# TaKeTube/TaKe

Measured on AMD Instinct MI355X. Metric: Msamples/s (camera paths/s: rays traced x spp / s), 1M-tri soup; weak scaling: 256 spp per GPU, higher is better.
Workload: dtype f64+f32; 1 GPU; procedural 1000000-triangle soup (diffuse materials) in 5-wall box + 1 quad area light, 1920x1080, 256 spp per GPU (256 total), max_depth 50, no Russian roulette, procedural sky env-map 2048x1024, importance-sampled (extension); parallelism=tile-row strips over 1 GPU(s), scene replicated, one gather

## Files before the change

### take_amd/csrc/tk_adaptive.h

```cpp
#pragma once
#include <cstdint>

#include "tk_integrate.h"

namespace tk {
namespace ad {

struct Rule {
    int32_t spp, min_spp, step_spp;
    double threshold, floor;
};

TK_HD double sample_value(double r, double g, double b) { return (r + g) + b; }
TK_HD void add_moments(double L, double &m1, double &m2) {
    m1 = m1 + L;
    m2 = m2 + L * L;
}

TK_HD double rel_error(int32_t n, double m1, double m2, double floor) {
    const double dn = (double)n;
    const double mean = m1 / dn;
    double v = m2 / dn - mean * mean;
    v = v > 0.0 ? v : 0.0;
    return tk_sqrt(v / (dn - 1.0)) / (tk_fabs(mean) + floor);
// ... 27 lines not shown
        base[g] = prefix;
        prefix += bits_of(mask[g]);
    }
    return prefix;
}
TK_HD int32_t compact_dest(const uint64_t *mask, const int32_t *base, int64_t j) {
    return base[j / GROUP] + rank_below(mask[j / GROUP], (int)(j % GROUP));
}

inline int32_t compact_serial(const uint8_t *keep, const int32_t *list, int64_t n, int threads, uint64_t *mask, int32_t *base, int32_t *out) {
    const int64_t n_groups = groups_of(n);
    for (int64_t g = 0; g < n_groups; g++) {
        uint64_t m = 0;
        for (int l = 0; l < GROUP; l++)
            if (g * GROUP + l < n && keep[g * GROUP + l]) m |= 1ull << l;
        mask[g] = m;
    }
    int32_t prefix = 0;
    for (int t = 0; t < threads; t++) {
        int64_t lo, hi;
        scan_run(n_groups, threads, t, lo, hi);
        prefix = run_number(mask, lo, hi, prefix, base);
    }
    for (int64_t j = 0; j < n; j++)
        if (kept(mask[j / GROUP], (int)(j % GROUP))) out[compact_dest(mask, base, j)] = listed(list, j);
    return prefix;
}

#if defined(__HIPCC__)

template <class R>
__global__ void __launch_bounds__(BLOCK)
k_generate_list(DeviceScene<R> sc, RenderParams<R> rp, PathState<R> st, const int32_t *__restrict__ list, int32_t n_active, double inv_n_active,
                int32_t *queue, int64_t n) {
    for (int64_t j = (int64_t)blockIdx.x * BLOCK + threadIdx.x; j < n; j += (int64_t)gridDim.x * BLOCK) {
        uint32_t sample, idx;
        list_entry((uint32_t)j, (uint32_t)n_active, inv_n_active, sample, idx);
        const int64_t slot = slot_of(sample, list[idx], rp.npix);
        generate_path(sc, rp, st, slot);
        queue[j] = (int32_t)slot;
    }
}

template <class R>
__global__ void __launch_bounds__(BLOCK)
k_accumulate_stats(PathState<R> st, R *accum, int32_t *count, double *m1, double *m2, const int32_t *__restrict__ list, int32_t n_active,
                   int32_t npix, int32_t nb) {
    for (int32_t j = blockIdx.x * BLOCK + threadIdx.x; j < n_active; j += gridDim.x * BLOCK) {
        const int32_t p = listed(list, j);
        R r = accum[3 * (int64_t)p], g = accum[3 * (int64_t)p + 1], b = accum[3 * (int64_t)p + 2];
        double s1 = m1[p], s2 = m2[p];
        for (int s = 0; s < nb; s++) {
            const int64_t slot = slot_of((uint32_t)s, p, npix);
            const R lr = st.R_(S_LX, slot), lg = st.R_(S_LY, slot), lb = st.R_(S_LZ, slot);
            r = r + lr;
            g = g + lg;
            b = b + lb;
            add_moments(sample_value((double)lr, (double)lg, (double)lb), s1, s2);
        }
        accum[3 * (int64_t)p] = r;
        accum[3 * (int64_t)p + 1] = g;
        accum[3 * (int64_t)p + 2] = b;
        m1[p] = s1, m2[p] = s2;
        count[p] += nb;
    }
}
__global__ void __launch_bounds__(BLOCK)
k_accumulate_stats_mixed(PathState<double> a, PathState<float> b, double *accum, int32_t *count, double *m1, double *m2,
                         const int32_t *__restrict__ list, int32_t n_active, int32_t npix, int32_t nb) {
    for (int32_t j = blockIdx.x * BLOCK + threadIdx.x; j < n_active; j += gridDim.x * BLOCK) {
        const int32_t p = listed(list, j);
        double r = accum[3 * (int64_t)p], g = accum[3 * (int64_t)p + 1], bl = accum[3 * (int64_t)p + 2];
        double s1 = m1[p], s2 = m2[p];
        for (int s = 0; s < nb; s++) {
            const int64_t slot = slot_of((uint32_t)s, p, npix);
            const bool conv = a.I_(S_CONV, slot) != 0;
            const float bx = b.R_(S_LX, slot), by = b.R_(S_LY, slot), bz = b.R_(S_LZ, slot);
            const double lr = a.R_(S_LX, slot) + (conv ? (double)bx : 0.0);
            const double lg = a.R_(S_LY, slot) + (conv ? (double)by : 0.0);
            const double lb = a.R_(S_LZ, slot) + (conv ? (double)bz : 0.0);
            r = r + lr;
            g = g + lg;
            bl = bl + lb;
            add_moments(sample_value(lr, lg, lb), s1, s2);
        }
        accum[3 * (int64_t)p] = r;
        accum[3 * (int64_t)p + 1] = g;
        accum[3 * (int64_t)p + 2] = bl;
        m1[p] = s1, m2[p] = s2;
        count[p] += nb;
    }
}

__global__ void __launch_bounds__(BLOCK)
k_adaptive_select(Rule rule, const int32_t *__restrict__ count, const double *__restrict__ m1, const double *__restrict__ m2,
                  const int32_t *__restrict__ list, int32_t n_active, uint64_t *mask) {
    const int64_t j = (int64_t)blockIdx.x * BLOCK + threadIdx.x;
    bool keep = false;
    if (j < n_active) {
        const int32_t p = listed(list, j);
        const int32_t n = count[p];
        keep = !stops(rule, n, rel_error(n, m1[p], m2[p], rule.floor));
    }
    const uint64_t m = __ballot(keep);
    if (lane_id() == 0 && j < n_active) mask[j / GROUP] = m;
}
__global__ void __launch_bounds__(SCAN_THREADS) k_compact_scan(const uint64_t *__restrict__ mask, int64_t n_groups, int32_t *base, int32_t *n_next) {
    __shared__ int32_t s_sum[SCAN_THREADS];
    int64_t lo, hi;
    scan_run(n_groups, SCAN_THREADS, (int)threadIdx.x, lo, hi);
    const int32_t sum = run_sum(mask, lo, hi);
    s_sum[threadIdx.x] = sum;
    __syncthreads();
    for (int off = 1; off < SCAN_THREADS; off <<= 1) {
        const int32_t v = (int)threadIdx.x >= off ? s_sum[threadIdx.x - off] : 0;
        __syncthreads();
        s_sum[threadIdx.x] += v;
        __syncthreads();
    }
    (void)run_number(mask, lo, hi, s_sum[threadIdx.x] - sum, base);
    if (threadIdx.x == SCAN_THREADS - 1) *n_next = s_sum[SCAN_THREADS - 1];
}
__global__ void __launch_bounds__(BLOCK)
k_compact_scatter(const int32_t *__restrict__ list, const uint64_t *__restrict__ mask, const int32_t *__restrict__ base, int32_t n_active,
                  int32_t *next) {
    for (int64_t j = (int64_t)blockIdx.x * BLOCK + threadIdx.x; j < n_active; j += (int64_t)gridDim.x * BLOCK)
        if (kept(mask[j / GROUP], (int)(j % GROUP))) next[compact_dest(mask, base, j)] = listed(list, j);
}

template <class R>
__global__ void __launch_bounds__(BLOCK)
k_resolve_adaptive(const R *__restrict__ accum, const int32_t *__restrict__ count, const double *__restrict__ m1, const double *__restrict__ m2, R *out,
                   int32_t *count_out, double *m1_out, double *m2_out, int32_t width, int32_t n_local_rows) {
// ... 19 lines not shown
```

### take_amd/csrc/tk_integrate.h

```cpp
#pragma once

#include "tk_shade.h"

namespace tk {

template <class R> struct RenderParams {
    int32_t width, height;
    int32_t n_local_rows;
    int32_t npix;
    int32_t strip_first, strip_stride;
    int32_t spp;
    int32_t s0;
    int32_t spb;
    int32_t max_depth;
    int32_t integrator;
    uint64_t seed;
    R ray_eps;
    double inv_npix, inv_width;
};

TK_HD void divmod_u31(uint32_t n, uint32_t d, double inv_d, uint32_t &q, uint32_t &r) {
    if (inv_d == 0.0) {
        q = n / d, r = n % d;
        return;
// ... 5 lines not shown
}
template <class R> TK_HD void slot_pixel(const RenderParams<R> &rp, int64_t slot, int &sl, int &lr, int &x) {
    uint32_t q, p, row, col;
    divmod_u31((uint32_t)slot, (uint32_t)rp.npix, rp.inv_npix, q, p);
    divmod_u31(p, (uint32_t)rp.width, rp.inv_width, row, col);
    sl = (int)q, lr = (int)row, x = (int)col;
}

constexpr int TILE_ROWS = 4;

template <class R> TK_HD int local_row_to_y(const RenderParams<R> &rp, int lr) {
    return (rp.strip_first + (lr / TILE_ROWS) * rp.strip_stride) * TILE_ROWS + (lr % TILE_ROWS);
}

template <class R> TK_HD Rng path_rng(const RenderParams<R> &rp, int64_t slot, uint32_t ctr) {
    int sl, lr, x;
    slot_pixel(rp, slot, sl, lr, x);
    const int y = local_row_to_y(rp, lr);
    Rng r;
    r.key = rng_key(rp.seed, (uint64_t)y * (uint64_t)rp.width + (uint64_t)x, (uint64_t)(rp.s0 + sl));
    r.ctr = ctr;
    return r;
}

constexpr uint32_t CAMERA_DRAWS = 2;
template <class R> TK_HD Vec3<R> camera_dir(const CameraRec<R> &c, const RenderParams<R> &rp, int64_t slot) {
    int sl, lr, x;
    slot_pixel(rp, slot, sl, lr, x);
    const int y = local_row_to_y(rp, lr);
    Rng rng = path_rng(rp, slot, 0);
    const R ry = random_real<R>(rng);
    const R rx = random_real<R>(rng);
    return normalize(ld3(c.u) * ((R(x) + rx) / R(c.width) - R(0.5)) * c.viewport_width +
                     ld3(c.v) * ((R(y) + ry) / R(c.height) - R(0.5)) * c.viewport_height - ld3(c.w));
}
template <class R>
TK_HD void generate_path(const DeviceScene<R> &sc, const RenderParams<R> &rp, const PathState<R> &st, int64_t slot) {
    const CameraRec<R> &c = sc.cam;
    const Vec3<R> d = camera_dir(c, rp, slot);
    Rng rng = path_rng(rp, slot, 0);
    rng.ctr = CAMERA_DRAWS;
    st.R_(S_OX, slot) = c.lookfrom[0];
    st.R_(S_OY, slot) = c.lookfrom[1];
    st.R_(S_OZ, slot) = c.lookfrom[2];
    st.R_(S_DX, slot) = d.x;
    st.R_(S_DY, slot) = d.y;
    st.R_(S_DZ, slot) = d.z;
    st.R_(S_TX, slot) = R(1);
    st.R_(S_TY, slot) = R(1);
    st.R_(S_TZ, slot) = R(1);
    st.R_(S_LX, slot) = R(0);
    st.R_(S_LY, slot) = R(0);
    st.R_(S_LZ, slot) = R(0);
    st.I_(S_CTR, slot) = (int32_t)rng.ctr;
    st.I_(S_FLAGS, slot) = 0;
    st.I_(S_OCC, slot) = -1;
    st.I_(S_CONV, slot) = 0;
}

constexpr uint32_t REQ_EXTEND = 1, REQ_SHADOW = 2;
constexpr int TAG_ANY = -1;
constexpr int TAG_MISS = TAKE_MAT_COUNT;

template <class R, int TAG = TAG_ANY, class ST = PathState<R>>
TK_HD uint32_t shade_path(const DeviceScene<R> &sc, const RenderParams<R> &rp, const ST &st, int64_t slot,
                          int k) {
    const int32_t hit_prim = st.I_(S_HIT, slot);
    const Vec3<R> ro{st.R_(S_OX, slot), st.R_(S_OY, slot), st.R_(S_OZ, slot)};
    const Vec3<R> rd{st.R_(S_DX, slot), st.R_(S_DY, slot), st.R_(S_DZ, slot)};
    Vec3<R> thr{st.R_(S_TX, slot), st.R_(S_TY, slot), st.R_(S_TZ, slot)};
    Vec3<R> rad{st.R_(S_LX, slot), st.R_(S_LY, slot), st.R_(S_LZ, slot)};
    if (k == 0) {
        thr = Vec3<R>{R(1), R(1), R(1)};
        rad = Vec3<R>{R(0), R(0), R(0)};
        if (sizeof(R) == 8) st.I_(S_CONV, slot) = 0;
    }
    const Vec3<R> bg = ld3(sc.background);
    const R nlights = R(sc.n_lights);
    const bool miss = (TAG == TAG_MISS) || hit_prim < 0;
    Isect<R> v{};
    bool alive = !miss;
    if (!miss) make_isect(sc, ro, rd, hit_prim, st.R_(S_HT, slot), st.R_(S_HU, slot), st.R_(S_HV, slot), v,
                            sc.inst_shade ? st.I_(S_INST, slot) : -1);

    if (k == 0) {
        if (miss) {
            rad = bg;
            if (sc.env.light >= 0) {
                R unused;
                rad = env_eval(sc, rd, unused);
            }
        } else if (v.area_light != -1) {
            const LightRec<R> &l = sc.lights[v.area_light];
            if (l.kind == 1) rad = rad + thr * ld3(l.intensity);
        }
    } else {
        const Vec3<R> FG{st.R_(S_FX, slot), st.R_(S_FY, slot), st.R_(S_FZ, slot)};
        const R pdf = st.R_(S_PDF, slot);
        const bool was_specular = (st.I_(S_FLAGS, slot) & FLAG_SPECULAR) != 0;
        if (miss && sc.env.light >= 0) {
            R env_pdf;
            const Vec3<R> L = env_eval(sc, rd, env_pdf);
            const R light_pdf = env_pdf / nlights;
            rad = rad + thr * (FG * L * (was_specular ? (R(1) / pdf) : (pdf / (light_pdf * light_pdf + pdf * pdf))));
            thr = thr * (FG / pdf);
        } else if (miss) {
            thr = thr * (FG / pdf);
            rad = rad + thr * bg;
        } else {
            Vec3<R> C2{R(0), R(0), R(0)};
            if (v.area_light != -1) {
                const LightRec<R> &l = sc.lights[v.area_light];
                const R d = length(v.pos - ro);
                const Vec3<R> light_dir = normalize(v.pos - ro);
                const R light_pdf =
                    light_pdf_area(l, v.pos, ro) * (d * d) / (tk_fmax(dot(-v.gn, light_dir), R(0)) * nlights);
                if (light_pdf <= R(0)) {
                    alive = false;
                } else if (l.kind == 1) {
                    C2 = FG * ld3(l.intensity) *
                         (was_specular ? (R(1) / pdf) : (pdf / (light_pdf * light_pdf + pdf * pdf)));
                }
            }
            if (alive) {
                rad = rad + thr * C2;
                thr = thr * (FG / pdf);
            }
        }
    }
// ... 62 lines not shown
                const Vec3<R> dir_out = normalize(rec.dir_out);
                if (rec.pdf > R(0)) {
                    st.R_(S_DX, slot) = dir_out.x;
                    st.R_(S_DY, slot) = dir_out.y;
                    st.R_(S_DZ, slot) = dir_out.z;
                    st.R_(S_FX, slot) = FG.x;
                    st.R_(S_FY, slot) = FG.y;
                    st.R_(S_FZ, slot) = FG.z;
                    st.R_(S_PDF, slot) = rec.pdf;
                    st.I_(S_FLAGS, slot) = is_specular ? FLAG_SPECULAR : 0;
                    req |= REQ_EXTEND;
                }
            }
        }
        st.R_(S_OX, slot) = v.pos.x;
        st.R_(S_OY, slot) = v.pos.y;
        st.R_(S_OZ, slot) = v.pos.z;
        st.I_(S_CTR, slot) = (int32_t)rng.ctr;
    }
    st.R_(S_TX, slot) = thr.x;
    st.R_(S_TY, slot) = thr.y;
    st.R_(S_TZ, slot) = thr.z;
    st.R_(S_LX, slot) = rad.x;
    st.R_(S_LY, slot) = rad.y;
    st.R_(S_LZ, slot) = rad.z;
    return req;
}

constexpr int32_t FLAG_LIGHT_BRANCH = 2;
constexpr int FLAG_ITER_SHIFT = 8;

template <class R, class G> TK_HD int sample_light_by_power(const DeviceScene<R> &sc, G &rng) {
    const R u = random_real<R>(rng);
    const int size = sc.n_lights;
    int lo = 0, hi = size + 1;
    while (lo < hi) {
        const int mid = (lo + hi) >> 1;
        if (sc.light_cdf[mid] > u) hi = mid;
        else lo = mid + 1;
    }
    const int off = lo - 1;
    return off < 0 ? 0 : (off > size - 1 ? size - 1 : off);
}

template <class R, int TAG = TAG_ANY, class ST = PathState<R>>
TK_HD uint32_t shade_path_alt(const DeviceScene<R> &sc, const RenderParams<R> &rp, const ST &st, int64_t slot,
                              int k) {
    const bool raw = rp.integrator == 1, power = rp.integrator == 3;
    const int32_t hit_prim = st.I_(S_HIT, slot);
    const Vec3<R> ro{st.R_(S_OX, slot), st.R_(S_OY, slot), st.R_(S_OZ, slot)};
    const Vec3<R> rd{st.R_(S_DX, slot), st.R_(S_DY, slot), st.R_(S_DZ, slot)};
    Vec3<R> thr{st.R_(S_TX, slot), st.R_(S_TY, slot), st.R_(S_TZ, slot)};
    Vec3<R> rad{st.R_(S_LX, slot), st.R_(S_LY, slot), st.R_(S_LZ, slot)};
    const Vec3<R> bg = ld3(sc.background);
    const R nlights = R(sc.n_lights);
    const bool miss = (TAG == TAG_MISS) || hit_prim < 0;
    Isect<R> v{};
    if (!miss) make_isect(sc, ro, rd, hit_prim, st.R_(S_HT, slot), st.R_(S_HU, slot), st.R_(S_HV, slot), v,
                            sc.inst_shade ? st.I_(S_INST, slot) : -1);
    const int32_t flags = st.I_(S_FLAGS, slot);
    int iter = flags >> FLAG_ITER_SHIFT;
    bool alive = true;
    if (k == 0) {
        iter = 0;
        if (miss) rad = bg, alive = false;
    } else {
        const Vec3<R> FG{st.R_(S_FX, slot), st.R_(S_FY, slot), st.R_(S_FZ, slot)};
        const R pdf = st.R_(S_PDF, slot);
        if (raw) {
            if (miss) rad = rad + thr * bg, alive = false;
        } else if (flags & FLAG_LIGHT_BRANCH) {
            if (miss) {
                if (power) rad = rad + thr * bg;
                alive = false;
            } else if (power && v.area_light == -1) {
                alive = false;
            } else {
                thr = thr * (FG / pdf);
            }
        } else {
            const bool was_specular = (flags & FLAG_SPECULAR) != 0;
            R p = (sc.n_lights == 0 || was_specular) ? pdf : R(0.5) * pdf;
            if (miss) {
                thr = thr * (FG / p);
                rad = rad + thr * bg;
                alive = false;
            } else {
                if (!was_specular && v.area_light != -1) {
                    const LightRec<R> &l = sc.lights[v.area_light];
                    const R d = length(v.pos - ro);
                    const Vec3<R> light_dir = normalize(v.pos - ro);
                    const R lpd = light_pdf_area(l, v.pos, ro) * (d * d);
                    const R light_pdf = power ? lpd * sc.light_pmf[v.area_light] / tk_fmax(dot(-v.gn, light_dir), R(0))
                                              : lpd / (tk_fmax(dot(-v.gn, light_dir), R(0)) * nlights);
                    if (light_pdf <= R(0)) alive = false;
                    else p = p + R(0.5) * light_pdf;
                }
                if (alive) thr = thr * (FG / p);
            }
        }
        iter++;
    }

    uint32_t req = 0;
    if (TAG != TAG_MISS && alive) {
        Rng rng = path_rng(rp, slot, (uint32_t)st.I_(S_CTR, slot));
// ... 60 lines not shown
```

### take_amd/csrc/tk_kernels.h

```cpp
#pragma once

#include <hip/hip_runtime.h>

#include "tk_integrate.h"
#include "tk_trace_quad.h"

namespace tk {

constexpr int BLOCK = 256;
constexpr int WAVE = 64;

__device__ __forceinline__ int lane_id() { return threadIdx.x & (WAVE - 1); }
__device__ __forceinline__ int mask_rank(uint64_t mask) {
    return __builtin_amdgcn_mbcnt_hi((uint32_t)(mask >> 32), __builtin_amdgcn_mbcnt_lo((uint32_t)mask, 0));
}
__device__ __forceinline__ void wave_append(bool want, int32_t value, int32_t *counter, int32_t *queue) {
    const uint64_t mask = __ballot(want);
    if (mask == 0) return;
    const int leader = __ffsll((unsigned long long)mask) - 1;
    int32_t base = 0;
    if (lane_id() == leader) base = atomicAdd(counter, (int32_t)__popcll(mask));
    base = __shfl(base, leader);
    if (want) queue[base + mask_rank(mask)] = value;
}

template <class R>
__global__ void __launch_bounds__(BLOCK)
k_generate(DeviceScene<R> sc, RenderParams<R> rp, PathState<R> st, int32_t *queue, int64_t n) {
    for (int64_t s = (int64_t)blockIdx.x * BLOCK + threadIdx.x; s < n; s += (int64_t)gridDim.x * BLOCK) {
        generate_path(sc, rp, st, s);
        queue[s] = (int32_t)s;
    }
}

template <class R> struct CameraIo : PathIo<R> {
    CameraRec<R> cam;
    RenderParams<R> rp;
    template <bool SHADOW> __device__ __forceinline__ void load(int32_t i, RayT<R> &ray, int32_t &tag) const {
        const int64_t slot = i;
        tag = i;
        const Vec3<R> d = camera_dir(cam, rp, slot);
        const PathState<R> &st = this->st;
        st.R_(S_OX, slot) = cam.lookfrom[0], st.R_(S_OY, slot) = cam.lookfrom[1], st.R_(S_OZ, slot) = cam.lookfrom[2];
        st.R_(S_DX, slot) = d.x, st.R_(S_DY, slot) = d.y, st.R_(S_DZ, slot) = d.z;
        ray = make_ray(cam.lookfrom[0], cam.lookfrom[1], cam.lookfrom[2], d.x, d.y, d.z, this->eps, Const<R>::inf());
    }
};
__global__ void __launch_bounds__(BLOCK) k_iota(int32_t *queue, int64_t n) {
    for (int64_t s = (int64_t)blockIdx.x * BLOCK + threadIdx.x; s < n; s += (int64_t)gridDim.x * BLOCK) queue[s] = (int32_t)s;
}

#ifndef TK_SHADE_RECORD
#define TK_SHADE_RECORD 1
#endif
template <class R> struct RecordView {
    union {
        mutable uint4 q[PATH_REC * sizeof(R) / 16];
        mutable R w[PATH_REC];
    };
    __device__ __forceinline__ RecordView() {}
    __device__ __forceinline__ R &R_(int c, int64_t) const { return w[c]; }
    __device__ __forceinline__ int32_t &I_(int c, int64_t) const { return *reinterpret_cast<int32_t *>(&w[c]); }
};
#ifndef TK_SHADE_WAVES_F32
#define TK_SHADE_WAVES_F32 5
#endif
#ifndef TK_SHADE_WAVES_F64
#define TK_SHADE_WAVES_F64 0
#endif
template <class R, int TAG, bool ALT> constexpr int shade_waves() {
    const bool lambert = TAG == 0 || TAG == 7 || TAG == 8 || TAG == 10 || TAG == 11;
    const int w = sizeof(R) == 4 ? ((lambert && !ALT) ? TK_SHADE_WAVES_F32 : 0) : TK_SHADE_WAVES_F64;
    return w > 0 ? w : 1;
}
template <class R, int TAG, bool ALT = false>
__global__ void __launch_bounds__(BLOCK, (shade_waves<R, TAG, ALT>()))
k_shade(DeviceScene<R> sc, RenderParams<R> rp, PathState<R> st, const int32_t *__restrict__ queue,
        const int32_t *__restrict__ n_ptr, const int32_t *__restrict__ tag_count, int32_t *next_queue,
        int32_t *n_next, int32_t *shadow_queue, int32_t *n_shadow, int k, unsigned long long *counters, float *to_f32) {
    int32_t begin = 0, n = *n_ptr;
    if (tag_count) {
        for (int t = 0; t < TAG; t++) begin += tag_count[t];
        n = tag_count[TAG];
    }
    if (blockIdx.x == 0 && threadIdx.x == 0) atomicAdd(&counters[C_BOUNCES], (unsigned long long)n);
    const int32_t i = blockIdx.x * BLOCK + threadIdx.x;
    if (blockIdx.x * BLOCK >= n) return;
    uint32_t req = 0;
    int32_t slot = 0;
    if (i < n) {
        slot = queue[begin + i];
#if TK_SHADE_RECORD
        if constexpr (sizeof(R) == 4) {
            RecordView<R> rv;
            const char *rec = (const char *)(st.r + (int64_t)slot * PATH_REC);
            asm volatile(
                "global_load_dwordx4 %0, %8, off\n\t"
                "global_load_dwordx4 %1, %8, off offset:16\n\t"
                "global_load_dwordx4 %2, %8, off offset:32\n\t"
                "global_load_dwordx4 %3, %8, off offset:48\n\t"
                "global_load_dwordx4 %4, %8, off offset:64\n\t"
                "global_load_dwordx4 %5, %8, off offset:80\n\t"
                "global_load_dwordx4 %6, %8, off offset:96\n\t"
                "global_load_dwordx4 %7, %8, off offset:112\n\t"
                "s_waitcnt vmcnt(0)"
                : "=&v"(rv.q[0]), "=&v"(rv.q[1]), "=&v"(rv.q[2]), "=&v"(rv.q[3]), "=&v"(rv.q[4]), "=&v"(rv.q[5]), "=&v"(rv.q[6]),
                  "=&v"(rv.q[7])
                : "v"(rec)
                : "memory");
            req = ALT ? shade_path_alt<R, TAG, RecordView<R>>(sc, rp, rv, (int64_t)slot, k)
                      : shade_path<R, TAG, RecordView<R>>(sc, rp, rv, (int64_t)slot, k);
            uint4 *out = (uint4 *)(st.r + (int64_t)slot * PATH_REC);
#pragma unroll
            for (int c = 0; c < PATH_REC / 4; c++) out[c] = rv.q[c];
        } else
#endif
#if TK_SHADE_RECORD
        if constexpr (sizeof(R) == 8) {
            RecordView<R> rv;
            const char *rec = (const char *)(st.r + (int64_t)slot * PATH_REC);
            asm volatile(
                "global_load_dwordx4 %0, %16, off\n\t"
                "global_load_dwordx4 %1, %16, off offset:16\n\t"
                "global_load_dwordx4 %2, %16, off offset:32\n\t"
                "global_load_dwordx4 %3, %16, off offset:48\n\t"
// ... 114 lines not shown
    for (int32_t i = lo; i < hi; i++) sum += hist[i];
    s_sum[threadIdx.x] = sum;
    __syncthreads();
    for (int off = 1; off < SORT_SCAN_THREADS; off <<= 1) {
        const int32_t v = threadIdx.x >= off ? s_sum[threadIdx.x - off] : 0;
        __syncthreads();
        s_sum[threadIdx.x] += v;
        __syncthreads();
    }
    int32_t run = s_sum[threadIdx.x] - sum;
    for (int32_t i = lo; i < hi; i++) {
        base[i] = run;
        run += hist[i];
    }
    __syncthreads();
    if (threadIdx.x < N_SORT_KEYS) {
        const int32_t first = threadIdx.x * n_waves, next = first + n_waves;
        const int32_t end = next < total ? base[next] : s_sum[SORT_SCAN_THREADS - 1];
        tag_count[threadIdx.x] = end - base[first];
    }
}
__global__ void __launch_bounds__(BLOCK)
k_sort_scatter(const int32_t *__restrict__ queue, const int32_t *__restrict__ n_ptr, const uint8_t *__restrict__ keys,
               const int32_t *__restrict__ base, int32_t *sorted) {
    const int32_t n = *n_ptr, n_waves = gridDim.x * (BLOCK / WAVE);
    const int32_t w = blockIdx.x * (BLOCK / WAVE) + threadIdx.x / WAVE;
    int32_t begin, end;
    sort_range(n, w, n_waves, begin, end);
    if (begin >= end) return;
    int32_t off[N_SORT_KEYS];
#pragma unroll
    for (int t = 0; t < N_SORT_KEYS; t++) off[t] = base[t * n_waves + w];
    for (int32_t i = begin + lane_id(); i < end + lane_id(); i += WAVE) {
        const bool valid = i < end;
        const int key = valid ? (int)keys[i] : -1;
        int32_t pos = 0;
#pragma unroll
        for (int t = 0; t < N_SORT_KEYS; t++) {
            const uint64_t m = __ballot(key == t);
            if (key == t) pos = off[t] + mask_rank(m);
            off[t] += (int32_t)__popcll(m);
        }
        if (valid) sorted[pos] = queue[i];
    }
}

template <class R>
__global__ void __launch_bounds__(BLOCK)
k_accumulate(PathState<R> st, R *accum, int32_t npix, int32_t spb) {
    for (int32_t p = blockIdx.x * BLOCK + threadIdx.x; p < npix; p += gridDim.x * BLOCK) {
        R r = accum[3 * (int64_t)p], g = accum[3 * (int64_t)p + 1], b = accum[3 * (int64_t)p + 2];
        for (int s = 0; s < spb; s++) {
            const int64_t slot = (int64_t)s * npix + p;
            r = r + st.R_(S_LX, slot);
            g = g + st.R_(S_LY, slot);
            b = b + st.R_(S_LZ, slot);
        }
        accum[3 * (int64_t)p] = r;
        accum[3 * (int64_t)p + 1] = g;
        accum[3 * (int64_t)p + 2] = b;
    }
}
__global__ void __launch_bounds__(BLOCK)
k_convert_state(PathState<double> a, PathState<float> b, const int32_t *__restrict__ queue, const int32_t *__restrict__ n_ptr) {
    const int32_t n = *n_ptr;
    for (int32_t i = blockIdx.x * BLOCK + threadIdx.x; i < n; i += gridDim.x * BLOCK) {
        const int64_t s = queue[i];
        constexpr int WORDS[] = {S_OX, S_OY, S_OZ, S_DX, S_DY, S_DZ, S_PDF, S_TX, S_TY, S_TZ, S_LX, S_LY, S_LZ, S_FX, S_FY, S_FZ};
#pragma unroll
        for (int w = 0; w < 16; w++) b.R_(WORDS[w], s) = (float)a.R_(WORDS[w], s);
        b.I_(S_CTR, s) = a.I_(S_CTR, s);
        b.I_(S_FLAGS, s) = a.I_(S_FLAGS, s);
        b.I_(S_OCC, s) = -1;
        a.R_(S_LX, s) = 0.0, a.R_(S_LY, s) = 0.0, a.R_(S_LZ, s) = 0.0;
        a.I_(S_CONV, s) = 1;
    }
}
__global__ void __launch_bounds__(BLOCK)
k_accumulate_mixed(PathState<double> a, PathState<float> b, double *accum, int32_t npix, int32_t spb) {
    for (int32_t p = blockIdx.x * BLOCK + threadIdx.x; p < npix; p += gridDim.x * BLOCK) {
        double r = accum[3 * (int64_t)p], g = accum[3 * (int64_t)p + 1], bl = accum[3 * (int64_t)p + 2];
        for (int s = 0; s < spb; s++) {
            const int64_t slot = (int64_t)s * npix + p;
            const bool conv = a.I_(S_CONV, slot) != 0;
            const float bx = b.R_(S_LX, slot), by = b.R_(S_LY, slot), bz = b.R_(S_LZ, slot);
            r = r + (a.R_(S_LX, slot) + (conv ? (double)bx : 0.0));
            g = g + (a.R_(S_LY, slot) + (conv ? (double)by : 0.0));
            bl = bl + (a.R_(S_LZ, slot) + (conv ? (double)bz : 0.0));
        }
        accum[3 * (int64_t)p] = r;
        accum[3 * (int64_t)p + 1] = g;
        accum[3 * (int64_t)p + 2] = bl;
    }
}
template <class R>
__global__ void __launch_bounds__(BLOCK)
k_resolve(const R *__restrict__ accum, R *out, int32_t width, int32_t n_local_rows, int32_t spp) {
    const int32_t npix = width * n_local_rows;
    const R inv = R(1) / R(spp);
    for (int32_t p = blockIdx.x * BLOCK + threadIdx.x; p < npix; p += gridDim.x * BLOCK) {
        const int lr = p / width, x = p % width;
        const int64_t o = 3 * ((int64_t)(n_local_rows - 1 - lr) * width + x);
        out[o] = accum[3 * (int64_t)p] * inv;
        out[o + 1] = accum[3 * (int64_t)p + 1] * inv;
        out[o + 2] = accum[3 * (int64_t)p + 2] * inv;
    }
}

__device__ __forceinline__ uint16_t exr_half_bits(float f) {
    const uint32_t u = __float_as_uint(f);
    const uint32_t sign = (u >> 16) & 0x8000u;
    const int32_t exp = (int32_t)((u >> 23) & 0xFFu);
    const uint32_t man = u & 0x7FFFFFu;
    const int32_t newexp = exp - 112;
    uint32_t out = 0;
    if (exp == 255) out = 0x7C00u | (man != 0 ? 0x200u : 0u);
    else if (exp != 0 && newexp >= 31) out = 0x7C00u;
    else if (exp != 0 && newexp > 0) out = (((uint32_t)newexp << 10) | (man >> 13)) + ((man >> 12) & 1u);
    else if (exp != 0 && 14 - newexp <= 24) {
        const uint32_t full = man | 0x800000u;
        const int sh = 14 - newexp;
        out = (full >> sh) + ((full >> (sh - 1)) & 1u);
    }
    return (uint16_t)(out | sign);
}
template <class R>
__global__ void __launch_bounds__(BLOCK) k_pack_exr(const R *__restrict__ rgb, int32_t width, int32_t height, uint16_t *out) {
    const int64_t total = (int64_t)width * height * 3;
    for (int64_t i = (int64_t)blockIdx.x * BLOCK + threadIdx.x; i < total; i += (int64_t)gridDim.x * BLOCK) {
        const int x = (int)(i % width);
        const int c = (int)((i / width) % 3);
        const int64_t y = i / ((int64_t)3 * width);
        out[i] = exr_half_bits((float)rgb[(y * width + x) * 3 + (2 - c)]);
    }
}

}

namespace tk {
enum DebugTable { TAB_MATERIAL = 0, TAB_LIGHT = 1, TAB_TEXTURE = 2, TAB_TO_WORLD = 3, TAB_HEMICOS = 4, TAB_BURLEY = 5 };
constexpr int TAB_RND = 8;
// ... 98 lines not shown
```

### take_amd/csrc/tk_scene.h

```cpp
#pragma once

#include "tk_common.h"

namespace tk {

constexpr int32_t CHILD_EMPTY = (int32_t)0x80000000;
constexpr int MAX_LEAF = 4;
constexpr int MAX_STACK_ENTRIES_W8 = 192;
constexpr int MAX_STACK_ENTRIES = 96;

TK_HD int32_t make_leaf(int32_t first, int32_t count) { return -(1 + first * MAX_LEAF + (count - 1)); }
TK_HD int32_t leaf_first(int32_t c) { return (-c - 1) / MAX_LEAF; }
TK_HD int32_t leaf_count(int32_t c) { return ((-c - 1) % MAX_LEAF) + 1; }
constexpr int32_t INSTANCE_WORD_END = -(1 << 30);
TK_HD int32_t make_instance_word(int32_t id) { return (int32_t)(0x80000001u + (uint32_t)id); }
TK_HD bool is_instance_word(int32_t c) { return c < INSTANCE_WORD_END && c != CHILD_EMPTY; }
TK_HD int32_t instance_of_word(int32_t c) { return (int32_t)((uint32_t)c - 0x80000001u); }

template <class R> struct alignas(16) NodeChild {
    R bmin[3];
    R bmax[3];
    int32_t child;
    int32_t pad;
};
// ... 94 lines not shown
};

template <class R> struct alignas(16) InstTrace {
    R inv[12];
    float grid_lo[3], grid_step[3];
    int32_t root_child;
    int32_t pad;
};
template <class R> struct alignas(16) InstShade {
    R fwd[9];
    int32_t material;
    int32_t tag;
    int32_t shape_base;
    int32_t pad;
};

template <class R> struct CameraRec {
    R u[3], v[3], w[3], lookfrom[3];
    R viewport_width, viewport_height;
    int32_t width, height;
};

template <class R> struct DeviceScene {
    const Node4<R> *nodes;
    const QNode4 *qnodes;
    const QNode8 *qnodes8;
    float grid_lo[3], grid_step[3];
    const PrimRec<R> *prims;
    int32_t root_child;
    int32_t n_nodes;
    const ShapeInfo *shapes;
    const MeshInfo *meshes;
    const int32_t *face_idx;
    const R *normals;
    const R *uvs;
    const MaterialRec<R> *materials;
    const ImageInfo *images;
    const R *texels;
    const InstTrace<R> *inst_trace;
    const InstShade<R> *inst_shade;
    int32_t n_instances;
    const LightRec<R> *lights;
    const R *light_pmf;
    const R *light_cdf;
    int32_t n_lights;
    int32_t n_shapes;
    R background[3];
    EnvMap<R> env;
    CameraRec<R> cam;
};

enum StateR {
    S_OX = 0, S_OY, S_OZ,
    S_DX, S_DY, S_DZ,
    S_HT, S_HU, S_HV,
    S_PDF = 12,
    S_TX, S_TY, S_TZ,
    S_LX, S_LY, S_LZ,
    S_ST,
    S_FX, S_FY, S_FZ,
    S_SX, S_SY, S_SZ,
    S_CX, S_CY, S_CZ,
    S_NUM_R = 29
};
enum StateI { S_HIT = 9, S_CTR = 10, S_FLAGS = 11, S_INST = 29, S_OCC = 30, S_CONV = 31, S_NUM_I = 6 };
constexpr int PATH_REC = 32;
constexpr int32_t FLAG_SPECULAR = 1;

template <class R> struct PathState {
    R *r;
    int64_t stride;
    TK_HD R &R_(int c, int64_t s) const { return r[s * PATH_REC + c]; }
    TK_HD int32_t &I_(int c, int64_t s) const { return *reinterpret_cast<int32_t *>(&r[s * PATH_REC + c]); }
};

enum QueueWord {
    Q_N_EXT0, Q_N_EXT1,
    Q_N_SHADOW,
    Q_HEAD_CLOSEST,
    Q_HEAD_SHADOW,
    Q_HEAD_SHADE,
    Q_NUM_WORDS = 16
};

enum CounterWord {
    C_NODE_VISITS, C_PRIM_TESTS, C_RAYS_CLOSEST, C_RAYS_SHADOW, C_BOUNCES, C_LEAF_VISITS, C_WAVE_NODE_STEPS,
    C_WAVE_LEAF_STEPS, C_WAIT_SLOTS, C_IDLE_SLOTS,
    C_RAYS_CLOSEST_TAIL,
    C_OCC_CACHE_HITS,
    C_NUM_WORDS = 12
};

}
```

### take_amd/csrc/tk_trace_quad.h

```cpp
#pragma once

#include <hip/hip_runtime.h>

#include <cstddef>

#include "tk_traverse.h"

namespace tk {

#ifndef TQ_GROUP
#define TQ_GROUP 1
#endif
#ifndef TQ_MIN_WAVES
#define TQ_MIN_WAVES (TQ_GROUP == 1 ? 5 : 6)
#endif
#ifndef TQ_INST_WAVES
#define TQ_INST_WAVES (TQ_MIN_WAVES - 1)
#endif
#ifndef TQ_F64_WAVES
#define TQ_F64_WAVES 4
#endif
#ifndef TQ_W8_WAVES
#define TQ_W8_WAVES 4
#endif
// ... 25 lines not shown
#define TQ_TIEBREAK 1
#endif
constexpr int TQ_BLOCK = 256;
constexpr int TQ_NODE_ITERS = TQ_NODE_ITERS_DEF;
constexpr uint32_t TQ_KEY_INVALID = 0x7FFFFFFFu;

typedef unsigned long long tq_entry;

__device__ __forceinline__ uint64_t tq_ballot(bool p) { return __builtin_amdgcn_ballot_w64(p); }
__device__ __forceinline__ int tq_less(uint32_t a, uint32_t b) { return (int)((a - b) >> 31); }

template <int CTRL> __device__ __forceinline__ int dpp_i(int v) {
    return __builtin_amdgcn_mov_dpp(v, CTRL, 0xf, 0xf, true);
}
template <int CTRL> __device__ __forceinline__ float dpp_f(float v) {
    return __int_as_float(dpp_i<CTRL>(__float_as_int(v)));
}
template <int CTRL> __device__ __forceinline__ double dpp_f(double v) {
    int lo = __double2loint(v), hi = __double2hiint(v);
    return __hiloint2double(dpp_i<CTRL>(hi), dpp_i<CTRL>(lo));
}
constexpr int QP_B0 = 0x00, QP_B1 = 0x55, QP_B2 = 0xAA, QP_B3 = 0xFF;
constexpr int QP_X1 = 0xB1;
constexpr int QP_EVEN = 0xA0, QP_ODD = 0xF5;
constexpr int QP_X2 = 0x4E;
struct StackSpill {
    tq_entry *base;
    int64_t stride;
};
__device__ __noinline__ void tq_spill_store(tq_entry *p, tq_entry e) { *p = e; }
__device__ __noinline__ tq_entry tq_spill_load(const tq_entry *p) { return *p; }

template <class R> struct PathIo {
    static constexpr bool UNIFORM_TMIN = true;
    const PrimRec<R> *prims;
    PathState<R> st;
    const int32_t *queue;
    R eps;
    __device__ __forceinline__ R tmin() const { return eps; }
    template <bool SHADOW> __device__ __forceinline__ void load(int32_t i, RayT<R> &ray, int32_t &tag) const {
        const int64_t slot = queue[i];
        tag = (int32_t)slot;
        reload<SHADOW>(slot, ray);
    }
    template <bool SHADOW> __device__ __forceinline__ void reload(int64_t slot, RayT<R> &ray) const {
        if (!SHADOW)
            ray = make_ray(st.R_(S_OX, slot), st.R_(S_OY, slot), st.R_(S_OZ, slot), st.R_(S_DX, slot), st.R_(S_DY, slot),
                           st.R_(S_DZ, slot), eps, Const<R>::inf());
        else
            ray = make_ray(st.R_(S_OX, slot), st.R_(S_OY, slot), st.R_(S_OZ, slot), st.R_(S_SX, slot), st.R_(S_SY, slot),
                           st.R_(S_SZ, slot), eps, st.R_(S_ST, slot));
    }
    __device__ __forceinline__ void store_hit(int64_t slot, int32_t prim, R t, R u, R v) const {
        st.I_(S_HIT, slot) = prim;
        st.R_(S_HT, slot) = t;
        st.R_(S_HU, slot) = u;
        st.R_(S_HV, slot) = v;
    }
    __device__ __forceinline__ void store_instance(int64_t slot, int32_t inst) const { st.I_(S_INST, slot) = inst; }
    static constexpr bool OCC_PROBE = true;
    __device__ __forceinline__ int32_t last_occluder(int64_t slot) const { return st.I_(S_OCC, slot); }
    __device__ __forceinline__ void set_last_occluder(int64_t slot, int32_t prim) const { st.I_(S_OCC, slot) = prim; }
    __device__ __forceinline__ void store_occlusion(int64_t slot, bool occluded) const {
        if (!occluded) {
            st.R_(S_LX, slot) = st.R_(S_LX, slot) + st.R_(S_CX, slot);
            st.R_(S_LY, slot) = st.R_(S_LY, slot) + st.R_(S_CY, slot);
            st.R_(S_LZ, slot) = st.R_(S_LZ, slot) + st.R_(S_CZ, slot);
        }
    }
};
template <class R> struct RayAoS {
    R org[3], tmin, dir[3], tmax;
};
template <class R> struct HitAoS;
template <> struct HitAoS<float> {
    int32_t shape_id;
    float t, u, v;
};
template <> struct HitAoS<double> {
    int32_t shape_id, reserved;
    double t, u, v;
};
template <class R> struct HookIo {
    static constexpr bool UNIFORM_TMIN = false;
    static constexpr bool OCC_PROBE = false;
    __device__ __forceinline__ int32_t last_occluder(int64_t) const { return -1; }
    __device__ __forceinline__ void set_last_occluder(int64_t, int32_t) const {}
    __device__ __forceinline__ R tmin() const { return R(0); }
    const PrimRec<R> *prims;
    const RayAoS<R> *rays;
    HitAoS<R> *hits;
    int32_t *occluded;
    const InstShade<R> *inst_shade;
    template <bool SHADOW> __device__ __forceinline__ void load(int32_t i, RayT<R> &ray, int32_t &tag) const {
        tag = i;
        reload<SHADOW>(i, ray);
    }
    template <bool SHADOW> __device__ __forceinline__ void reload(int64_t i, RayT<R> &ray) const {
        const RayAoS<R> q = rays[i];
        ray = make_ray(q.org[0], q.org[1], q.org[2], q.dir[0], q.dir[1], q.dir[2], q.tmin > R(0) ? q.tmin : R(0), q.tmax);
    }
    __device__ __forceinline__ void store_instance(int64_t i, int32_t inst) const {
        if (inst >= 0 && hits[i].shape_id >= 0) hits[i].shape_id += inst_shade[inst].shape_base;
    }
    __device__ __forceinline__ void store_hit(int64_t i, int32_t prim, R t, R u, R v) const {
        HitAoS<R> h{};
        h.shape_id = prim >= 0 ? prims[prim].shape_id : -1;
        h.t = prim >= 0 ? t : R(0);
        h.u = u;
        h.v = v;
        hits[i] = h;
    }
    __device__ __forceinline__ void store_occlusion(int64_t i, bool occ) const { occluded[i] = occ ? 1 : 0; }
};

template <int G, int W = 4> struct GroupGeom {
    static constexpr int LOG2 = G == 4 ? 2 : (G == 2 ? 1 : 0);
    static constexpr int CPL = 4 / G;
    static constexpr int GROUPS = TQ_BLOCK / G;
    static constexpr int PER_WAVE = 64 / G;
// ... 492 lines not shown
```

Measured before the change: 80.14 Msamples/s.

## Defer NEE radiance add via sign flag and repack path record for vector hit stores

When a shadow ray is unoccluded, the traversal kernel no longer does a read-modify-write of the radiance from the light contribution. It now writes a single negative word into the shadow-tmax slot as a pending flag, and shading and accumulation add the contribution later. The path-state record is reordered so that hit prim, t, u and v sit in one aligned quad and can be written with 128-bit stores. This cuts scattered memory traffic in the trace kernel, at the cost of extra conditional loads in shade and accumulate. A TAG 3 shading kernel also gets the capped f32 wave count.

```diff
diff --git a/take_amd/csrc/tk_adaptive.h b/take_amd/csrc/tk_adaptive.h
--- a/take_amd/csrc/tk_adaptive.h
+++ b/take_amd/csrc/tk_adaptive.h
@@ -103,7 +103,8 @@
         double s1 = m1[p], s2 = m2[p];
         for (int s = 0; s < nb; s++) {
             const int64_t slot = slot_of((uint32_t)s, p, npix);
-            const R lr = st.R_(S_LX, slot), lg = st.R_(S_LY, slot), lb = st.R_(S_LZ, slot);
+            R lr, lg, lb;
+            sample_radiance(st, slot, lr, lg, lb);
             r = r + lr;
             g = g + lg;
             b = b + lb;
@@ -126,10 +127,13 @@
         for (int s = 0; s < nb; s++) {
             const int64_t slot = slot_of((uint32_t)s, p, npix);
             const bool conv = a.I_(S_CONV, slot) != 0;
-            const float bx = b.R_(S_LX, slot), by = b.R_(S_LY, slot), bz = b.R_(S_LZ, slot);
-            const double lr = a.R_(S_LX, slot) + (conv ? (double)bx : 0.0);
-            const double lg = a.R_(S_LY, slot) + (conv ? (double)by : 0.0);
-            const double lb = a.R_(S_LZ, slot) + (conv ? (double)bz : 0.0);
+            float bx, by, bz;
+            double ax, ay, az;
+            sample_radiance(b, slot, bx, by, bz);
+            sample_radiance(a, slot, ax, ay, az);
+            const double lr = ax + (conv ? (double)bx : 0.0);
+            const double lg = ay + (conv ? (double)by : 0.0);
+            const double lb = az + (conv ? (double)bz : 0.0);
             r = r + lr;
             g = g + lg;
             bl = bl + lb;
diff --git a/take_amd/csrc/tk_integrate.h b/take_amd/csrc/tk_integrate.h
--- a/take_amd/csrc/tk_integrate.h
+++ b/take_amd/csrc/tk_integrate.h
@@ -81,6 +81,7 @@
     st.R_(S_LX, slot) = R(0);
     st.R_(S_LY, slot) = R(0);
     st.R_(S_LZ, slot) = R(0);
+    st.R_(S_ST, slot) = R(0);
     st.I_(S_CTR, slot) = (int32_t)rng.ctr;
     st.I_(S_FLAGS, slot) = 0;
     st.I_(S_OCC, slot) = -1;
@@ -103,7 +104,10 @@
         thr = Vec3<R>{R(1), R(1), R(1)};
         rad = Vec3<R>{R(0), R(0), R(0)};
         if (sizeof(R) == 8) st.I_(S_CONV, slot) = 0;
-    }
+    } else if (pending_nee(st.R_(S_ST, slot))) {
+        rad = rad + Vec3<R>{st.R_(S_CX, slot), st.R_(S_CY, slot), st.R_(S_CZ, slot)};
+    }
+    st.R_(S_ST, slot) = R(0);
     const Vec3<R> bg = ld3(sc.background);
     const R nlights = R(sc.n_lights);
     const bool miss = (TAG == TAG_MISS) || hit_prim < 0;
@@ -272,6 +276,10 @@
     const Vec3<R> rd{st.R_(S_DX, slot), st.R_(S_DY, slot), st.R_(S_DZ, slot)};
     Vec3<R> thr{st.R_(S_TX, slot), st.R_(S_TY, slot), st.R_(S_TZ, slot)};
     Vec3<R> rad{st.R_(S_LX, slot), st.R_(S_LY, slot), st.R_(S_LZ, slot)};
+    if (k >= 1 && pending_nee(st.R_(S_ST, slot))) {
+        rad = rad + Vec3<R>{st.R_(S_CX, slot), st.R_(S_CY, slot), st.R_(S_CZ, slot)};
+        st.R_(S_ST, slot) = R(0);
+    }
     const Vec3<R> bg = ld3(sc.background);
     const R nlights = R(sc.n_lights);
     const bool miss = (TAG == TAG_MISS) || hit_prim < 0;
diff --git a/take_amd/csrc/tk_kernels.h b/take_amd/csrc/tk_kernels.h
--- a/take_amd/csrc/tk_kernels.h
+++ b/take_amd/csrc/tk_kernels.h
@@ -70,7 +70,8 @@
 #endif
 template <class R, int TAG, bool ALT> constexpr int shade_waves() {
     const bool lambert = TAG == 0 || TAG == 7 || TAG == 8 || TAG == 10 || TAG == 11;
-    const int w = sizeof(R) == 4 ? ((lambert && !ALT) ? TK_SHADE_WAVES_F32 : 0) : TK_SHADE_WAVES_F64;
+    const bool capped = lambert || TAG == 3;
+    const int w = sizeof(R) == 4 ? ((capped && !ALT) ? TK_SHADE_WAVES_F32 : 0) : TK_SHADE_WAVES_F64;
     return w > 0 ? w : 1;
 }
 template <class R, int TAG, bool ALT = false>
@@ -291,9 +292,11 @@
         R r = accum[3 * (int64_t)p], g = accum[3 * (int64_t)p + 1], b = accum[3 * (int64_t)p + 2];
         for (int s = 0; s < spb; s++) {
             const int64_t slot = (int64_t)s * npix + p;
-            r = r + st.R_(S_LX, slot);
-            g = g + st.R_(S_LY, slot);
-            b = b + st.R_(S_LZ, slot);
+            R lr, lg, lb;
+            sample_radiance(st, slot, lr, lg, lb);
+            r = r + lr;
+            g = g + lg;
+            b = b + lb;
         }
         accum[3 * (int64_t)p] = r;
         accum[3 * (int64_t)p + 1] = g;
@@ -311,6 +314,7 @@
         b.I_(S_CTR, s) = a.I_(S_CTR, s);
         b.I_(S_FLAGS, s) = a.I_(S_FLAGS, s);
         b.I_(S_OCC, s) = -1;
+        b.R_(S_ST, s) = 0.0f;
         a.R_(S_LX, s) = 0.0, a.R_(S_LY, s) = 0.0, a.R_(S_LZ, s) = 0.0;
         a.I_(S_CONV, s) = 1;
     }
@@ -322,10 +326,13 @@
         for (int s = 0; s < spb; s++) {
             const int64_t slot = (int64_t)s * npix + p;
             const bool conv = a.I_(S_CONV, slot) != 0;
-            const float bx = b.R_(S_LX, slot), by = b.R_(S_LY, slot), bz = b.R_(S_LZ, slot);
-            r = r + (a.R_(S_LX, slot) + (conv ? (double)bx : 0.0));
-            g = g + (a.R_(S_LY, slot) + (conv ? (double)by : 0.0));
-            bl = bl + (a.R_(S_LZ, slot) + (conv ? (double)bz : 0.0));
+            float bx, by, bz;
+            double ax, ay, az;
+            sample_radiance(b, slot, bx, by, bz);
+            sample_radiance(a, slot, ax, ay, az);
+            r = r + (ax + (conv ? (double)bx : 0.0));
+            g = g + (ay + (conv ? (double)by : 0.0));
+            bl = bl + (az + (conv ? (double)bz : 0.0));
         }
         accum[3 * (int64_t)p] = r;
         accum[3 * (int64_t)p + 1] = g;
diff --git a/take_amd/csrc/tk_scene.h b/take_amd/csrc/tk_scene.h
--- a/take_amd/csrc/tk_scene.h
+++ b/take_amd/csrc/tk_scene.h
@@ -170,18 +170,20 @@
 
 enum StateR {
     S_OX = 0, S_OY, S_OZ,
+    S_ST,
     S_DX, S_DY, S_DZ,
-    S_HT, S_HU, S_HV,
-    S_PDF = 12,
+    S_SX = 8, S_SY, S_SZ,
+    S_HT = 13, S_HU, S_HV,
+    S_PDF,
     S_TX, S_TY, S_TZ,
     S_LX, S_LY, S_LZ,
-    S_ST,
     S_FX, S_FY, S_FZ,
-    S_SX, S_SY, S_SZ,
     S_CX, S_CY, S_CZ,
     S_NUM_R = 29
 };
-enum StateI { S_HIT = 9, S_CTR = 10, S_FLAGS = 11, S_INST = 29, S_OCC = 30, S_CONV = 31, S_NUM_I = 6 };
+enum StateI { S_CTR = 7, S_FLAGS = 11, S_HIT = 12, S_INST = 29, S_OCC = 30, S_CONV = 31, S_NUM_I = 6 };
+static_assert(S_ST == 3 && S_DZ == 6 && S_SZ == 10 && S_HV == 15 && S_PDF == 16 && S_CZ == 28, "the record's word order");
+template <class R> TK_HD bool pending_nee(R st_word) { return st_word < R(0); }
 constexpr int PATH_REC = 32;
 constexpr int32_t FLAG_SPECULAR = 1;
 
@@ -191,6 +193,13 @@
     TK_HD R &R_(int c, int64_t s) const { return r[s * PATH_REC + c]; }
     TK_HD int32_t &I_(int c, int64_t s) const { return *reinterpret_cast<int32_t *>(&r[s * PATH_REC + c]); }
 };
+
+template <class R> TK_HD void sample_radiance(const PathState<R> &st, int64_t slot, R &x, R &y, R &z) {
+    const bool nee = pending_nee(st.R_(S_ST, slot));
+    const R cx = st.R_(S_CX, slot), cy = st.R_(S_CY, slot), cz = st.R_(S_CZ, slot);
+    x = st.R_(S_LX, slot), y = st.R_(S_LY, slot), z = st.R_(S_LZ, slot);
+    x = nee ? x + cx : x, y = nee ? y + cy : y, z = nee ? z + cz : z;
+}
 
 enum QueueWord {
     Q_N_EXT0, Q_N_EXT1,
diff --git a/take_amd/csrc/tk_trace_quad.h b/take_amd/csrc/tk_trace_quad.h
--- a/take_amd/csrc/tk_trace_quad.h
+++ b/take_amd/csrc/tk_trace_quad.h
@@ -101,10 +101,15 @@
                            st.R_(S_SZ, slot), eps, st.R_(S_ST, slot));
     }
     __device__ __forceinline__ void store_hit(int64_t slot, int32_t prim, R t, R u, R v) const {
-        st.I_(S_HIT, slot) = prim;
-        st.R_(S_HT, slot) = t;
-        st.R_(S_HU, slot) = u;
-        st.R_(S_HV, slot) = v;
+        static_assert(S_HIT == 12 && S_HT == 13 && S_HU == 14 && S_HV == 15, "quad 3 of the record");
+        uint4 *out = (uint4 *)(st.r + slot * PATH_REC + S_HIT);
+        if constexpr (sizeof(R) == 4) {
+            out[0] = make_uint4((uint32_t)prim, __float_as_uint(t), __float_as_uint(u), __float_as_uint(v));
+        } else {
+            out[0] = make_uint4((uint32_t)prim, (uint32_t)prim, (uint32_t)__double2loint(t), (uint32_t)__double2hiint(t));
+            out[1] = make_uint4((uint32_t)__double2loint(u), (uint32_t)__double2hiint(u), (uint32_t)__double2loint(v),
+                                (uint32_t)__double2hiint(v));
+        }
     }
     __device__ __forceinline__ void store_instance(int64_t slot, int32_t inst) const { st.I_(S_INST, slot) = inst; }
     static constexpr bool OCC_PROBE = true;
@@ -112,9 +117,10 @@
     __device__ __forceinline__ void set_last_occluder(int64_t slot, int32_t prim) const { st.I_(S_OCC, slot) = prim; }
     __device__ __forceinline__ void store_occlusion(int64_t slot, bool occluded) const {
         if (!occluded) {
-            st.R_(S_LX, slot) = st.R_(S_LX, slot) + st.R_(S_CX, slot);
-            st.R_(S_LY, slot) = st.R_(S_LY, slot) + st.R_(S_CY, slot);
-            st.R_(S_LZ, slot) = st.R_(S_LZ, slot) + st.R_(S_CZ, slot);
+            int32_t m;
+            if constexpr (sizeof(R) == 4) asm volatile("v_mov_b32 %0, 0xbf800000" : "=v"(m));
+            else asm volatile("v_mov_b32 %0, 0xbff00000" : "=v"(m));
+            reinterpret_cast<int32_t *>(st.r + slot * PATH_REC + S_ST)[sizeof(R) / 4 - 1] = m;
         }
     }
 };
```

Result: no change. 80.57 Msamples/s (median of 6 runs) (+0.5%).
